# JOBR0/PerceiverIO_Pytorch

Measured on AMD Instinct MI355X. Metric: samples/sec PerceiverIO fwd (ImageNet-224, 512x1024 latents, 8 blocks x 6 self-attends), higher is better.
Workload: dtype f16; 1 GPU; imagenet224 ClassificationPerceiver (conv+Fourier prep -> encoder 3136x322->512x1024, 8x6 SA -> decoder 1000 queries -> final Linear), all rows computed; batch_per_gpu=32, global_batch=32, precision_policy=fp16x2w/fp16sd/fp16x2af, parallelism=dp1 (batch sharded, all-gather of logits), launch=one HIP graph replay per step

## Files before the change

include/pio_hip.h:

```cpp
#ifndef PIO_HIP_H
#define PIO_HIP_H

#include <stddef.h>
#include <stdint.h>

#ifdef __cplusplus
extern "C" {
#endif

#define PIO_VERSION 100

enum {
    PIO_OK = 0,
    PIO_E_SHAPE = -1,
    PIO_E_ALIGN = -2,
    PIO_E_ARCH = -3,
    PIO_E_WORKSPACE = -4,
    PIO_E_LAUNCH = -5,
    PIO_E_ARG = -6,
    PIO_E_RANGE = -7
};

enum { PIO_DT_F16 = 0, PIO_DT_BF16 = 1 };


typedef struct pio_linear_t {
    const void *w_hi;
    const void *w_lo;
    const float *bias;
    int32_t n;
    int32_t k;
    int32_t lo_row0;
} pio_linear_t;

typedef struct pio_layernorm_t {
    const float *gamma;
    const float *beta;
    int32_t c;
    float eps;
} pio_layernorm_t;

typedef struct pio_attention_t {
    pio_linear_t q, k, v, o;
    int32_t heads;
    int32_t dk, dv;
    int32_t dkp, dvp;
    int32_t q_in, k_in, v_in, out;
    int32_t dtype;
    int32_t act_split;
    pio_linear_t qk;
    pio_linear_t qkv;
    pio_linear_t kq, vo;
} pio_attention_t;

typedef struct pio_mlp_t {
    pio_linear_t fc1, fc2;
    int32_t in, hidden, out;
    int32_t dtype;
    int32_t act_split;
} pio_mlp_t;

typedef struct pio_ln_fold_t {
    pio_linear_t qkv;
    const float *qkv_c;
    pio_linear_t fc1;
    const float *fc1_c;
    int32_t *range_flag;
} pio_ln_fold_t;

typedef struct pio_self_attention_t {
    pio_layernorm_t ln1, ln2;
    pio_attention_t attn;
    pio_mlp_t mlp;
    pio_ln_fold_t fold;
} pio_self_attention_t;

typedef struct pio_cross_attention_t {
    pio_layernorm_t ln_q, ln_kv, ln2;
    pio_attention_t attn;
    pio_mlp_t mlp;
    int32_t use_query_residual;
} pio_cross_attention_t;

typedef struct pio_tensor3_t {
    const float *data;
    int64_t stride_b;
    int64_t stride_t;
    int32_t B, T, C;
} pio_tensor3_t;

int pio_version(void);
int pio_arch_ok(void);
const char *pio_error_string(int code);

#define PIO_PROF_CLASSES 9
int pio_prof_begin(int32_t max_records);
int pio_prof_end(double *ms, double *flops, double *bytes, int64_t *launches);

int pio_ln_fold_enable(int on);

int pio_gemm_kernel_override(int which);

int pio_stream_create_cu_mask(void **stream, const uint32_t *mask, uint32_t words);
int pio_stream_destroy(void *stream);
int pio_set_cu_budget(int32_t n_cu);

int32_t pio_pad8(int32_t c);
int32_t pio_padc(int32_t c);
size_t pio_packed_weight_bytes(int32_t out, int32_t in, int32_t row_heads, int32_t col_heads);
int pio_pack_linear(const float *w, const float *bias, int32_t out, int32_t in, int64_t ldw,
                    int32_t row_heads, int32_t col_heads, void *dst_hi, void *dst_lo, float *dst_bias,
                    int32_t dst_row0, int32_t k_pad, int32_t dtype, void *stream);

int pio_layernorm_cast(const pio_tensor3_t *x, const pio_layernorm_t *ln, void *y, void *y_lo, int32_t c_pad,
                       int32_t dtype, void *stream);

int pio_layernorm_cast_cat(const pio_tensor3_t *x1, const pio_tensor3_t *x2, const pio_layernorm_t *ln, void *y,
                           void *y_lo, int32_t c_pad, int32_t dtype, void *stream);

int pio_bn_relu_maxpool_tokens(const float *x, const float *scale, const float *shift, float *y, int32_t B, int32_t C,
                               int32_t H, int32_t W, int32_t pad_top, int32_t pad_left, void *stream);

typedef struct pio_gemm_t {
    const void *A, *B;
    const void *A_lo, *B_lo;
    void *C;
    void *C_lo;
    int32_t M, N, K;
    int64_t lda, ldb, ldc;
    int32_t batch, nh;
    int64_t sAb, sAh, sBb, sBh, sCb, sCh;
    const float *bias;
    int32_t bias_mode;
    int32_t act;
    float alpha;
    const float *R;
    int64_t ldr, r_stride_b;
    int32_t r_rows_per_batch;
    int32_t out_f32;
    int32_t n_store;
    int32_t dtype;
    void *X16;
    int64_t ld16;
    float *row_part;
    const float *ln_part;
    const float *ln_c;
    float ln_eps;
    void *X16_lo;
    const void *R16_hi, *R16_lo;
    int32_t b_lo_n0;
    int32_t *range_flag;
    int32_t ln_slots;
    int32_t row_slot_w;
} pio_gemm_t;
int pio_gemm_nt(const pio_gemm_t *g, void *stream);

int pio_softmax_rows(const float *S, int64_t lds, void *P, void *P_lo, int64_t ldp, int32_t B, int32_t H,
                     int32_t Tq, int32_t Tk, float scale, const uint8_t *kv_mask, const uint8_t *q_mask,
                     const uint8_t *full_mask, const float *bias, int32_t dtype, void *stream);

int pio_flash_attention(int32_t dtype, int32_t dkp, int32_t dvp, int32_t dk, const void *Q, const void *K, const void *V,
                        void *O, int32_t B, int32_t H, int32_t Tq, int32_t Tk, int64_t ldq, int64_t ldk, int64_t ldv,
                        int64_t ldo, int64_t sQb, int64_t sKb, int64_t sVb, int64_t sOb, int32_t v_rowmajor, void *stream);

size_t pio_flash_attention_pair_workspace_bytes(int32_t dkp, int32_t dvp, int32_t B, int32_t H, int32_t Tq, int32_t Tk);
int pio_flash_attention_pair(int32_t dtype, int32_t dkp, int32_t dvp, int32_t dk, const void *Q, const void *Q_lo,
                             const void *K, const void *K_lo, const void *V, void *O, void *O_lo, int32_t B, int32_t H,
                             int32_t Tq, int32_t Tk, int64_t ldq, int64_t ldk, int64_t ldv, int64_t ldo, int64_t sQb,
                             int64_t sKb, int64_t sVb, int64_t sOb, int32_t v_rowmajor, const uint8_t *kv_mask,
                             const uint8_t *q_mask, int32_t core, void *workspace, size_t workspace_bytes, void *stream);

size_t pio_attention_workspace_bytes(const pio_attention_t *a, int32_t B, int32_t Tq, int32_t Tk);
int pio_attention_fwd(const pio_attention_t *a, const pio_tensor3_t *inputs_q, const pio_tensor3_t *inputs_k,
                      const pio_tensor3_t *inputs_v, const uint8_t *kv_mask, const uint8_t *q_mask,
                      const uint8_t *full_mask, const float *attention_bias, float *out, float *probs_out,
                      void *workspace, size_t workspace_bytes, void *stream);

size_t pio_mlp_workspace_bytes(const pio_mlp_t *m, int64_t rows);
int pio_mlp_fwd(const pio_mlp_t *m, const pio_tensor3_t *x, float *out, void *workspace,
                size_t workspace_bytes, void *stream);

typedef struct pio_call_opts_t {
    int32_t ln_fold;
    int32_t cu_budget;
} pio_call_opts_t;

size_t pio_self_attention_workspace_bytes(const pio_self_attention_t *s, int32_t B, int32_t N);
int pio_self_attention_fwd(const pio_self_attention_t *s, const pio_tensor3_t *x, const uint8_t *kv_mask,
                           const uint8_t *q_mask, const uint8_t *full_mask, const float *attention_bias,
                           float *out, float *probs_out, void *workspace, size_t workspace_bytes, void *stream);

int pio_self_attention_fwd_opts(const pio_self_attention_t *s, const pio_tensor3_t *x, const uint8_t *kv_mask,
                                const uint8_t *q_mask, const uint8_t *full_mask, const float *attention_bias,
                                float *out, float *probs_out, void *workspace, size_t workspace_bytes, void *stream,
                                const pio_call_opts_t *opts);

size_t pio_cross_attention_workspace_bytes(const pio_cross_attention_t *c, int32_t B, int32_t Tq, int32_t Tk);
int pio_cross_attention_fwd(const pio_cross_attention_t *c, const pio_tensor3_t *inputs_q,
                            const pio_tensor3_t *inputs_kv, const uint8_t *kv_mask, const uint8_t *q_mask,
                            const uint8_t *full_mask, const float *attention_bias, float *out, float *probs_out,
                            void *workspace, size_t workspace_bytes, void *stream);

size_t pio_encoder_workspace_bytes(const pio_cross_attention_t *cross, const pio_self_attention_t *layers,
                                   int32_t L, int32_t B, int32_t M, int32_t N);
int pio_encoder_fwd(const pio_cross_attention_t *cross, const pio_self_attention_t *layers, int32_t L,
                    int32_t num_blocks, const pio_tensor3_t *inputs, const pio_tensor3_t *latents,
                    const uint8_t *input_mask, float *out, void *workspace, size_t workspace_bytes,
                    void *stream);

int pio_encoder_fwd_split(const pio_cross_attention_t *cross, const pio_self_attention_t *layers, int32_t L,
                          int32_t num_blocks, const pio_tensor3_t *inputs, const pio_tensor3_t *inputs_tail,
                          const pio_tensor3_t *latents, const uint8_t *input_mask, float *out, void *workspace,
                          size_t workspace_bytes, void *stream);

int pio_encoder_fwd_blocks(const pio_cross_attention_t *cross, const pio_self_attention_t *layers, int32_t L,
                           int32_t num_blocks, int32_t per_block, const pio_tensor3_t *inputs,
                           const pio_tensor3_t *inputs_tail, const pio_tensor3_t *latents, const uint8_t *input_mask,
                           float *out, void *workspace, size_t workspace_bytes, void *stream);

int pio_encoder_fwd_opts(const pio_cross_attention_t *cross, const pio_self_attention_t *layers, int32_t L,
                         int32_t num_blocks, int32_t per_block, const pio_tensor3_t *inputs,
                         const pio_tensor3_t *inputs_tail, const pio_tensor3_t *latents, const uint8_t *input_mask,
                         float *out, void *workspace, size_t workspace_bytes, void *stream,
                         const pio_call_opts_t *opts);

size_t pio_decoder_workspace_bytes(const pio_cross_attention_t *cross, const pio_linear_t *final_layer,
                                   int32_t B, int32_t Q, int32_t N);
int pio_decoder_fwd(const pio_cross_attention_t *cross, const pio_linear_t *final_layer, int32_t final_out,
                    const pio_tensor3_t *query, const pio_tensor3_t *latents, const uint8_t *query_mask,
                    float *out, void *workspace, size_t workspace_bytes, void *stream);

size_t pio_decoder_qcache_bytes(const pio_cross_attention_t *cross, int32_t Bq, int32_t Q);
int pio_decoder_fwd_qcache(const pio_cross_attention_t *cross, const pio_linear_t *final_layer, int32_t final_out,
                           const pio_tensor3_t *query, const pio_tensor3_t *latents, const uint8_t *query_mask,
                           float *out, void *workspace, size_t workspace_bytes, void *stream, void *q16_hi,
                           void *q16_lo, int32_t q16_valid);

int pio_decoder_fwd_split(const pio_cross_attention_t *cross, const pio_linear_t *final_layer, int32_t final_out,
                          const pio_tensor3_t *query, const pio_tensor3_t *query_tail, const pio_tensor3_t *latents,
                          const uint8_t *query_mask, float *out, void *workspace, size_t workspace_bytes, void *stream);

#ifdef __cplusplus
}
#endif
#endif
```

perceiverio_pytorch_amd/_lib.py:

```python
from __future__ import annotations

import ctypes as C
import os
import subprocess

_HERE = os.path.dirname(os.path.abspath(__file__))
LIB_PATH = os.environ.get("PIO_LIB_PATH", os.path.join(_HERE, "libpio_hip.so"))
CSRC = os.path.join(_HERE, "csrc")

PIO_DT_F16 = 0
PIO_DT_BF16 = 1

PIO_OK = 0
_ERRORS = {-1: "PIO_E_SHAPE", -2: "PIO_E_ALIGN", -3: "PIO_E_ARCH", -4: "PIO_E_WORKSPACE", -5: "PIO_E_LAUNCH",
           -6: "PIO_E_ARG", -7: "PIO_E_RANGE"}


class PioError(RuntimeError):
    pass


class Linear(C.Structure):
    _fields_ = [("w_hi", C.c_void_p), ("w_lo", C.c_void_p), ("bias", C.c_void_p), ("n", C.c_int32), ("k", C.c_int32),
                ("lo_row0", C.c_int32)]


class LayerNorm(C.Structure):
    _fields_ = [("gamma", C.c_void_p), ("beta", C.c_void_p), ("c", C.c_int32), ("eps", C.c_float)]


class Attention(C.Structure):
    _fields_ = [("q", Linear), ("k", Linear), ("v", Linear), ("o", Linear), ("heads", C.c_int32),
                ("dk", C.c_int32), ("dv", C.c_int32), ("dkp", C.c_int32), ("dvp", C.c_int32),
                ("q_in", C.c_int32), ("k_in", C.c_int32), ("v_in", C.c_int32), ("out", C.c_int32), ("dtype", C.c_int32),
                ("act_split", C.c_int32), ("qk", Linear), ("qkv", Linear), ("kq", Linear), ("vo", Linear)]


class Mlp(C.Structure):
    _fields_ = [("fc1", Linear), ("fc2", Linear), ("in_", C.c_int32), ("hidden", C.c_int32), ("out", C.c_int32),
                ("dtype", C.c_int32), ("act_split", C.c_int32)]


class LnFold(C.Structure):
    _fields_ = [("qkv", Linear), ("qkv_c", C.c_void_p), ("fc1", Linear), ("fc1_c", C.c_void_p),
                ("range_flag", C.c_void_p)]


class SelfAttention(C.Structure):
    _fields_ = [("ln1", LayerNorm), ("ln2", LayerNorm), ("attn", Attention), ("mlp", Mlp), ("fold", LnFold)]


class CrossAttention(C.Structure):
    _fields_ = [("ln_q", LayerNorm), ("ln_kv", LayerNorm), ("ln2", LayerNorm), ("attn", Attention), ("mlp", Mlp),
                ("use_query_residual", C.c_int32)]


class Tensor3(C.Structure):
    _fields_ = [("data", C.c_void_p), ("stride_b", C.c_int64), ("stride_t", C.c_int64), ("B", C.c_int32),
                ("T", C.c_int32), ("C", C.c_int32)]


class CallOpts(C.Structure):
    _fields_ = [("ln_fold", C.c_int32), ("cu_budget", C.c_int32)]


class Gemm(C.Structure):
    _fields_ = [("A", C.c_void_p), ("B", C.c_void_p), ("A_lo", C.c_void_p), ("B_lo", C.c_void_p), ("C", C.c_void_p),
                ("C_lo", C.c_void_p),
                ("M", C.c_int32), ("N", C.c_int32), ("K", C.c_int32),
                ("lda", C.c_int64), ("ldb", C.c_int64), ("ldc", C.c_int64),
                ("batch", C.c_int32), ("nh", C.c_int32),
                ("sAb", C.c_int64), ("sAh", C.c_int64), ("sBb", C.c_int64), ("sBh", C.c_int64),
                ("sCb", C.c_int64), ("sCh", C.c_int64),
                ("bias", C.c_void_p), ("bias_mode", C.c_int32), ("act", C.c_int32), ("alpha", C.c_float),
                ("R", C.c_void_p), ("ldr", C.c_int64), ("r_stride_b", C.c_int64),
                ("r_rows_per_batch", C.c_int32), ("out_f32", C.c_int32), ("n_store", C.c_int32),
                ("dtype", C.c_int32),
                ("X16", C.c_void_p), ("ld16", C.c_int64), ("row_part", C.c_void_p), ("ln_part", C.c_void_p),
                ("ln_c", C.c_void_p), ("ln_eps", C.c_float),
                ("X16_lo", C.c_void_p), ("R16_hi", C.c_void_p), ("R16_lo", C.c_void_p), ("b_lo_n0", C.c_int32),
                ("range_flag", C.c_void_p), ("ln_slots", C.c_int32), ("row_slot_w", C.c_int32)]


P = C.POINTER
_vp, _i32, _i64, _sz, _f = C.c_void_p, C.c_int32, C.c_int64, C.c_size_t, C.c_float
SIGNATURES = {
    "pio_version": (C.c_int, []),
    "pio_arch_ok": (C.c_int, []),
    "pio_error_string": (C.c_char_p, [C.c_int]),
    "pio_prof_begin": (C.c_int, [_i32]),
    "pio_prof_end": (C.c_int, [P(C.c_double), P(C.c_double), P(C.c_double), P(C.c_int64)]),
    "pio_pad8": (_i32, [_i32]),
    "pio_padc": (_i32, [_i32]),
    "pio_gemm_kernel_override": (C.c_int, [C.c_int]),
    "pio_ln_fold_enable": (C.c_int, [C.c_int]),
    "pio_stream_create_cu_mask": (C.c_int, [P(_vp), P(C.c_uint32), C.c_uint32]),
    "pio_stream_destroy": (C.c_int, [_vp]),
    "pio_set_cu_budget": (C.c_int, [_i32]),
    "pio_packed_weight_bytes": (_sz, [_i32, _i32, _i32, _i32]),
    "pio_pack_linear": (C.c_int, [_vp, _vp, _i32, _i32, _i64, _i32, _i32, _vp, _vp, _vp, _i32, _i32, _i32, _vp]),
    "pio_layernorm_cast": (C.c_int, [P(Tensor3), P(LayerNorm), _vp, _vp, _i32, _i32, _vp]),
    "pio_layernorm_cast_cat": (C.c_int, [P(Tensor3), P(Tensor3), P(LayerNorm), _vp, _vp, _i32, _i32, _vp]),
    "pio_bn_relu_maxpool_tokens": (C.c_int, [_vp, _vp, _vp, _vp, _i32, _i32, _i32, _i32, _i32, _i32, _vp]),
    "pio_gemm_nt": (C.c_int, [P(Gemm), _vp]),
    "pio_softmax_rows": (C.c_int, [_vp, _i64, _vp, _vp, _i64, _i32, _i32, _i32, _i32, _f, _vp, _vp, _vp, _vp, _i32, _vp]),
    "pio_flash_attention": (C.c_int, [_i32, _i32, _i32, _i32, _vp, _vp, _vp, _vp, _i32, _i32, _i32, _i32, _i64, _i64, _i64,
                                      _i64, _i64, _i64, _i64, _i64, _i32, _vp]),
    "pio_flash_attention_pair_workspace_bytes": (_sz, [_i32, _i32, _i32, _i32, _i32, _i32]),
    "pio_flash_attention_pair": (C.c_int, [_i32, _i32, _i32, _i32, _vp, _vp, _vp, _vp, _vp, _vp, _vp, _i32, _i32, _i32, _i32,
                                           _i64, _i64, _i64, _i64, _i64, _i64, _i64, _i64, _i32, _vp, _vp, _i32, _vp, _sz,
                                           _vp]),
    "pio_attention_workspace_bytes": (_sz, [P(Attention), _i32, _i32, _i32]),
    "pio_attention_fwd": (C.c_int, [P(Attention), P(Tensor3), P(Tensor3), P(Tensor3), _vp, _vp, _vp, _vp, _vp, _vp,
                                    _vp, _sz, _vp]),
    "pio_mlp_workspace_bytes": (_sz, [P(Mlp), _i64]),
    "pio_mlp_fwd": (C.c_int, [P(Mlp), P(Tensor3), _vp, _vp, _sz, _vp]),
    "pio_self_attention_workspace_bytes": (_sz, [P(SelfAttention), _i32, _i32]),
    "pio_self_attention_fwd": (C.c_int, [P(SelfAttention), P(Tensor3), _vp, _vp, _vp, _vp, _vp, _vp, _vp, _sz, _vp]),
    "pio_self_attention_fwd_opts": (C.c_int, [P(SelfAttention), P(Tensor3), _vp, _vp, _vp, _vp, _vp, _vp, _vp, _sz, _vp,
                                              P(CallOpts)]),
    "pio_cross_attention_workspace_bytes": (_sz, [P(CrossAttention), _i32, _i32, _i32]),
    "pio_cross_attention_fwd": (C.c_int, [P(CrossAttention), P(Tensor3), P(Tensor3), _vp, _vp, _vp, _vp, _vp, _vp,
                                          _vp, _sz, _vp]),
    "pio_encoder_workspace_bytes": (_sz, [P(CrossAttention), P(SelfAttention), _i32, _i32, _i32, _i32]),
    "pio_encoder_fwd": (C.c_int, [P(CrossAttention), P(SelfAttention), _i32, _i32, P(Tensor3), P(Tensor3), _vp, _vp,
                                  _vp, _sz, _vp]),
    "pio_encoder_fwd_split": (C.c_int, [P(CrossAttention), P(SelfAttention), _i32, _i32, P(Tensor3), P(Tensor3),
                                        P(Tensor3), _vp, _vp, _vp, _sz, _vp]),
    "pio_encoder_fwd_blocks": (C.c_int, [P(CrossAttention), P(SelfAttention), _i32, _i32, _i32, P(Tensor3), P(Tensor3),
                                         P(Tensor3), _vp, _vp, _vp, _sz, _vp]),
    "pio_encoder_fwd_opts": (C.c_int, [P(CrossAttention), P(SelfAttention), _i32, _i32, _i32, P(Tensor3), P(Tensor3),
                                       P(Tensor3), _vp, _vp, _vp, _sz, _vp, P(CallOpts)]),
    "pio_decoder_workspace_bytes": (_sz, [P(CrossAttention), P(Linear), _i32, _i32, _i32]),
    "pio_decoder_fwd": (C.c_int, [P(CrossAttention), P(Linear), _i32, P(Tensor3), P(Tensor3), _vp, _vp, _vp, _sz,
                                  _vp]),
    "pio_decoder_qcache_bytes": (_sz, [P(CrossAttention), _i32, _i32]),
    "pio_decoder_fwd_qcache": (C.c_int, [P(CrossAttention), P(Linear), _i32, P(Tensor3), P(Tensor3), _vp, _vp, _vp, _sz,
                                         _vp, _vp, _vp, _i32]),
    "pio_decoder_fwd_split": (C.c_int, [P(CrossAttention), P(Linear), _i32, P(Tensor3), P(Tensor3), P(Tensor3), _vp, _vp, _vp,
                                        _sz, _vp]),
}

_lib = None


def build(verbose: bool = False) -> str:
    out = subprocess.run(["make", "-C", CSRC, "-j8"], capture_output=True, text=True)
    if verbose or out.returncode:
        print(out.stdout[-4000:])
        print(out.stderr[-4000:])
    if out.returncode:
        raise PioError("building libpio_hip.so failed")
    return LIB_PATH


def lib() -> C.CDLL:
    global _lib
    if _lib is None:
        if not os.path.exists(LIB_PATH):
            raise PioError(f"{LIB_PATH} is missing: run `python -c 'import __graft_entry__ as g; g.build()'` "
                           "(there is no CPU / eager fallback for the PerceiverIO hot path)")
        l = C.CDLL(LIB_PATH)
        for name, (res, args) in SIGNATURES.items():
            fn = getattr(l, name)
            fn.restype = res
            fn.argtypes = args
        _lib = l
    return _lib


def check(code: int, what: str = "") -> None:
    if code != PIO_OK:
        raise PioError(f"{what}: {_ERRORS.get(code, code)}")
```

perceiverio_pytorch_amd/csrc/pio_flash.hip:

```cpp
#include <stdio.h>
#include <stdlib.h>

#include <type_traits>

#include "pio_internal.h"

namespace pio {

#ifndef PIO_FLASH_DEFAULT_VARIANT
#define PIO_FLASH_DEFAULT_VARIANT 0
#endif

struct FlashParams {
    const void *Q, *K, *VT;
    void *O;
    int Tq, Tk, H, nqt;
    int64_t ldq, ldk, ldvt, ldo;
    int64_t sQb, sKb, sVb, sOb;
    float scale_log2;
    int o_rows16;
    const void *Q_lo, *K_lo;
    void *O_lo;
};

static __device__ __attribute__((aligned(16))) uint32_t g_zero_chunk_f[4] = {0, 0, 0, 0};

template <int DV>
__device__ __forceinline__ int vrow_swz(int r) {
    if constexpr (DV == 128) return ((r & 3) << 2) | ((r >> 2) & 3);
    else if constexpr (DV == 64) return ((r >> 1) & 1) << 2;
    else return 0;
}

template <int DT, int DK, int DV, bool VROW, int NW, int KS = 1, bool QK_PAIR = false>
__global__ __launch_bounds__(NW * 64, NW >= 8 ? 1 : 2) void flash_attn_kernel(const FlashParams p) {
    static_assert(!QK_PAIR || (DK == 32 && DT == PIO_DT_F16), "pair-operand Q K^T: the DK = 32 fp16 instantiations");
    typedef typename Op<DT>::T T;
    typedef typename Op<DT>::V8 V8;
    typedef typename Op<DT>::V4 V4;
    typedef short tr4 __attribute__((__vector_size__(4 * sizeof(short))));
    static_assert(!VROW || DV == 128 || DV == 64 || DV == 32 || DV == 160, "row-major V: swizzles exist for these widths");
    constexpr int KT = 64;
    constexpr int K_TILE = KT * DK * 2;
    constexpr int K_STG = QK_PAIR ? 2 * K_TILE : K_TILE;
    constexpr int V_TILE = DV * KT * 2;
    constexpr int KCPR = DK / 8;
    constexpr int KRPB = 16 / KCPR;
    constexpr int K_PIECES = K_TILE / 1024;
    constexpr int V_PIECES = V_TILE / 1024;
    constexpr int NDT = DV / 32;
    constexpr int NQS = DK / 16;
    constexpr int OROW = DV * 2 + 16;
    static_assert(KS == 1 || ((KS == 2 || KS == 4) && NW == 4 * KS), "key split: KS groups of four waves");
    constexpr int NWQ = NW / KS;
    constexpr int MRG = KS > 1 ? (KS - 1) * NWQ * 64 * (NDT * 16 + 2) * 4 : 0;
    constexpr int RING = 2 * KS * (K_STG + V_TILE), OSTG = NW * 32 * OROW;
    constexpr int SM0 = RING > OSTG ? RING : OSTG;
    __shared__ __attribute__((aligned(16))) char smem[SM0 > MRG ? SM0 : MRG];

    const int tid = threadIdx.x;
    const int lane = tid & 63;
    const int wave = __builtin_amdgcn_readfirstlane(tid >> 6);
    const int r32 = lane & 31, hh = lane >> 5;
    int bid = blockIdx.x;
    const int nblk = gridDim.x;
    if ((nblk & 7) == 0) bid = (bid & 7) * (nblk >> 3) + (bid >> 3);
    const int qt = bid % p.nqt, bh = bid / p.nqt;
    const int b = bh / p.H, h = bh % p.H;
    const int qb = KS == 1 ? wave : wave % NWQ, kh = KS == 1 ? 0 : wave / NWQ;
    const int q0 = qt * (NWQ * 32) + qb * 32;

    const T *Qg = (const T *)p.Q + b * p.sQb + (int64_t)h * DK;
    const T *Kg = (const T *)p.K + b * p.sKb + (int64_t)h * DK;
    const T *Vg = (const T *)p.VT + b * p.sVb + (VROW ? (int64_t)h * DV : (int64_t)h * DV * p.ldvt);
    const T *zsrc = (const T *)g_zero_chunk_f;
    const T *Klg = nullptr;
    if constexpr (QK_PAIR) Klg = (const T *)p.K_lo + b * p.sKb + (int64_t)h * DK;

    V8 qf[NQS];
    V8 ql[QK_PAIR ? NQS : 1];

    const int ntiles_all = (p.Tk + KT - 1) / KT;
    const int ntiles = ntiles_all / KS;
    const int tile0 = kh * ntiles;

    auto stage = [&](int kt, int buf) {
        char *kb = smem + (buf * KS + kh) * (K_STG + V_TILE);
        char *vb = kb + K_STG;
        const int k0 = (tile0 + kt) * KT;
        for (int pc = qb; pc < K_PIECES; pc += NWQ) {
            const int row = pc * (64 / KCPR) + lane / KCPR;
            const int slot = lane % KCPR;
            const int c = slot ^ ((row / KRPB) & (KCPR - 1));
            int key = k0 + row;
            key = key < p.Tk ? key : p.Tk - 1;
            const T *src = Kg + (int64_t)key * p.ldk + c * 8;
            __builtin_amdgcn_global_load_lds((const __attribute__((address_space(1))) void *)src,
                                             (__attribute__((address_space(3))) void *)(kb + pc * 1024), 16, 0, 0);
            if constexpr (QK_PAIR)
                __builtin_amdgcn_global_load_lds(
                    (const __attribute__((address_space(1))) void *)(Klg + (int64_t)key * p.ldk + c * 8),
                    (__attribute__((address_space(3))) void *)(kb + K_TILE + pc * 1024), 16, 0, 0);
        }
        if constexpr (VROW) {
            constexpr int VCPR = DV / 8;
            for (int pc = qb; pc < V_PIECES; pc += NWQ) {
                const int idx = pc * 64 + lane;
                const int row = idx / VCPR;
                const int slot = idx - row * VCPR;
                const int c = slot ^ vrow_swz<DV>(row);
                int key = k0 + row;
                key = key < p.Tk ? key : p.Tk - 1;
                const T *src = Vg + (int64_t)key * p.ldvt + c * 8;
                __builtin_amdgcn_global_load_lds((const __attribute__((address_space(1))) void *)src,
                                                 (__attribute__((address_space(3))) void *)(vb + pc * 1024), 16, 0,
                                                 0);
            }
        } else
        for (int pc = qb; pc < V_PIECES; pc += NWQ) {
            const int row = pc * 8 + (lane >> 3);
            const int slot = lane & 7;
            const int c = slot ^ ((row >> 1) & 7);
            const int kcol = k0 + c * 8;
            const T *src = (kcol < p.ldvt) ? Vg + (int64_t)row * p.ldvt + kcol : zsrc;
            __builtin_amdgcn_global_load_lds((const __attribute__((address_space(1))) void *)src,
                                             (__attribute__((address_space(3))) void *)(vb + pc * 1024), 16, 0, 0);
        }
    };

    f32x16 oacc[NDT];
#pragma unroll
    for (int i = 0; i < NDT; ++i)
#pragma unroll
        for (int j = 0; j < 16; ++j) oacc[i][j] = 0.f;
    float m_run = -INFINITY;
    float l_run = 0.f;

    int k_off[2];
#pragma unroll
    for (int t = 0; t < 2; ++t) k_off[t] = (32 * t + r32) * (DK * 2);
    const int k_swz = (r32 / KRPB) & (KCPR - 1);
    const int v_swz = (r32 >> 1) & 7;

    stage(0, 0);
    {
        int q = q0 + r32;
        q = q < p.Tq ? q : p.Tq - 1;
        const T *qrow = Qg + (int64_t)q * p.ldq + 8 * hh;
#pragma unroll
        for (int s = 0; s < NQS; ++s) qf[s] = *(const V8 *)(qrow + 16 * s);
        if constexpr (QK_PAIR) {
            const T *lrow = (const T *)p.Q_lo + b * p.sQb + (int64_t)h * DK + (int64_t)q * p.ldq + 8 * hh;
#pragma unroll
            for (int s = 0; s < NQS; ++s) ql[s] = *(const V8 *)(lrow + 16 * s);
        }
    }
    for (int kt = 0; kt < ntiles; ++kt) {
        asm volatile("s_waitcnt vmcnt(0)" ::: "memory");
        __syncthreads();
        if (kt + 1 < ntiles) stage(kt + 1, (kt + 1) & 1);
        const char *kb = smem + ((kt & 1) * KS + kh) * (K_STG + V_TILE);
        const char *vb = kb + K_STG;

        f32x16 sacc[2];
#pragma unroll
        for (int t = 0; t < 2; ++t) {
#pragma unroll
            for (int j = 0; j < 16; ++j) sacc[t][j] = 0.f;
            if constexpr (QK_PAIR) {
                V8 kh_f[NQS], kl_f[NQS];
#pragma unroll
                for (int s = 0; s < NQS; ++s) {
                    const int chunk = (2 * s + hh) ^ k_swz;
                    kh_f[s] = *(const V8 *)(kb + k_off[t] + chunk * 16);
                    kl_f[s] = *(const V8 *)(kb + K_TILE + k_off[t] + chunk * 16);
                }
#pragma unroll
                for (int s = 0; s < NQS; ++s) sacc[t] = Op<DT>::mfma32(kl_f[s], qf[s], sacc[t]);
#pragma unroll
                for (int s = 0; s < NQS; ++s) sacc[t] = Op<DT>::mfma32(kh_f[s], ql[s], sacc[t]);
#pragma unroll
                for (int s = 0; s < NQS; ++s) sacc[t] = Op<DT>::mfma32(kh_f[s], qf[s], sacc[t]);
            } else
#pragma unroll
            for (int s = 0; s < NQS; ++s) {
                const int chunk = (2 * s + hh) ^ k_swz;
                const V8 kf = *(const V8 *)(kb + k_off[t] + chunk * 16);
                sacc[t] = Op<DT>::mfma32(kf, qf[s], sacc[t]);
            }
        }
        const bool tail = KS == 1 && (kt == ntiles - 1) && (p.Tk % KT != 0);
        float mx = -INFINITY;
        if (tail) {
#pragma unroll
            for (int t = 0; t < 2; ++t)
#pragma unroll
                for (int i = 0; i < 16; ++i) {
                    const int key = (tile0 + kt) * KT + 32 * t + (i & 3) + 8 * (i >> 2) + 4 * hh;
                    if (key >= p.Tk) sacc[t][i] = -INFINITY;
                }
        }
#pragma unroll
        for (int t = 0; t < 2; ++t)
#pragma unroll
            for (int i = 0; i < 16; ++i) mx = fmaxf(mx, sacc[t][i]);
        mx = fmaxf(mx, __shfl_xor(mx, 32, 64)) * p.scale_log2;
        const float m_new = fmaxf(m_run, mx);
        const float alpha = __builtin_amdgcn_exp2f(m_run - m_new);
        m_run = m_new;
        float psum = 0.f;
#pragma unroll
        for (int t = 0; t < 2; ++t)
#pragma unroll
            for (int i = 0; i < 16; ++i) {
                const float e = __builtin_amdgcn_exp2f(fmaf(sacc[t][i], p.scale_log2, -m_new));
                sacc[t][i] = e;
                psum += e;
            }
        l_run = l_run * alpha + psum;
        if (__builtin_amdgcn_ballot_w64(alpha != 1.0f) != 0) {
#pragma unroll
            for (int d = 0; d < NDT; ++d)
#pragma unroll
                for (int j = 0; j < 16; ++j) oacc[d][j] *= alpha;
        }

        V8 pf[2][2];
#pragma unroll
        for (int t = 0; t < 2; ++t)
#pragma unroll
            for (int s = 0; s < 2; ++s)
#pragma unroll
                for (int j = 0; j < 8; ++j) pf[t][s][j] = Op<DT>::from_f32(sacc[t][8 * s + j]);

#pragma unroll
        for (int d = 0; d < NDT; ++d) {
            const char *vrow = vb + (32 * d + r32) * 128;
#pragma unroll
            for (int t = 0; t < 2; ++t)
#pragma unroll
                for (int s = 0; s < 2; ++s) {
                    V4 lo, hi;
                    if constexpr (VROW) {
                        const int q4 = (lane & 15) >> 2, p4 = lane & 3, g1 = (lane >> 4) & 1;
                        const int chunk = d * 4 + 2 * g1 + (p4 >> 1);
#pragma unroll
                        for (int jj = 0; jj < 2; ++jj) {
                            const int key = 32 * t + 16 * s + 8 * jj + 4 * hh + q4;
                            const int f = vrow_swz<DV>(key);
                            const char *a = vb + key * (DV * 2) + ((chunk ^ f) << 4) + 8 * (p4 & 1);
                            const tr4 r = __builtin_amdgcn_ds_read_tr16_b64_v4i16(
                                (__attribute__((address_space(3))) tr4 *)a);
                            if (jj == 0) lo = __builtin_bit_cast(V4, r);
                            else hi = __builtin_bit_cast(V4, r);
                        }
                    } else {
                        const int g = 8 * t + 4 * s + hh;
                        lo = *(const V4 *)(vrow + ((((g >> 1)) ^ v_swz) << 4) + (g & 1) * 8);
                        hi = *(const V4 *)(vrow + ((((g + 2) >> 1) ^ v_swz) << 4) + (g & 1) * 8);
                    }
                    V8 vf;
#pragma unroll
                    for (int j = 0; j < 4; ++j) {
                        vf[j] = lo[j];
                        vf[4 + j] = hi[j];
                    }
                    oacc[d] = Op<DT>::mfma32(vf, pf[t][s], oacc[d]);
                }
        }
    }

    if constexpr (KS > 1) {
        __syncthreads();
        constexpr int MW = NDT * 16 + 2;
        if (kh > 0) {
            float *mg = (float *)smem + (size_t)(((kh - 1) * NWQ + qb) * 64 + lane) * MW;
#pragma unroll
            for (int d = 0; d < NDT; ++d)
#pragma unroll
                for (int j = 0; j < 16; ++j) mg[d * 16 + j] = oacc[d][j];
            mg[NDT * 16] = m_run;
            mg[NDT * 16 + 1] = l_run;
        }
        __syncthreads();
        if (kh == 0) {
#pragma unroll
            for (int part = 1; part < KS; ++part) {
                const float *mg = (const float *)smem + (size_t)(((part - 1) * NWQ + qb) * 64 + lane) * MW;
                const float m1 = mg[NDT * 16], l1 = mg[NDT * 16 + 1];
                const float m = fmaxf(m_run, m1);
                const float a0 = __builtin_amdgcn_exp2f(m_run - m), a1 = __builtin_amdgcn_exp2f(m1 - m);
#pragma unroll
                for (int d = 0; d < NDT; ++d)
#pragma unroll
                    for (int j = 0; j < 16; ++j) oacc[d][j] = oacc[d][j] * a0 + mg[d * 16 + j] * a1;
                l_run = l_run * a0 + l1 * a1;
                m_run = m;
            }
        }
    }
    const float l_tot = l_run + __shfl_xor(l_run, 32, 64);
    const float inv = 1.0f / l_tot;
    if (p.o_rows16) {
        __syncthreads();
        if (kh != 0) return;
        char *const ost = smem + qb * (32 * OROW);
        char *const orow = ost + r32 * OROW;
#pragma unroll
        for (int d = 0; d < NDT; ++d)
#pragma unroll
            for (int g4 = 0; g4 < 4; ++g4) {
                V4 o;
#pragma unroll
                for (int j = 0; j < 4; ++j) o[j] = Op<DT>::from_f32(oacc[d][4 * g4 + j] * inv);
                *(V4 *)(orow + (32 * d + 8 * g4 + 4 * hh) * 2) = o;
            }
        constexpr int CPR = DV / 8;
        T *const og = (T *)p.O + b * p.sOb + (int64_t)h * DV;
#pragma unroll
        for (int idx0 = 0; idx0 < 32 * CPR; idx0 += 64) {
            const int idx = idx0 + lane;
            const int row = idx / CPR, ch = idx % CPR;
            if (idx < 32 * CPR && q0 + row < p.Tq)
                *(V8 *)(og + (int64_t)(q0 + row) * p.ldo + ch * 8) = *(const V8 *)(ost + row * OROW + ch * 16);
        }
        return;
    }
    const int q = q0 + r32;
    if (q < p.Tq && kh == 0) {
        T *orow = (T *)p.O + b * p.sOb + (int64_t)q * p.ldo + (int64_t)h * DV;
#pragma unroll
        for (int d = 0; d < NDT; ++d)
#pragma unroll
            for (int g4 = 0; g4 < 4; ++g4) {
                V4 o;
#pragma unroll
                for (int j = 0; j < 4; ++j) o[j] = Op<DT>::from_f32(oacc[d][4 * g4 + j] * inv);
                *(V4 *)(orow + 32 * d + 8 * g4 + 4 * hh) = o;
                if constexpr (QK_PAIR) {
                    if (p.O_lo) {
                        V4 l;
#pragma unroll
                        for (int j = 0; j < 4; ++j)
                            l[j] = Op<DT>::from_f32(oacc[d][4 * g4 + j] * inv - Op<DT>::to_f32(o[j]));
                        *(V4 *)((T *)p.O_lo + (orow - (T *)p.O) + 32 * d + 8 * g4 + 4 * hh) = l;
                    }
                }
            }
    }
}

#ifdef PIO_EXPERIMENTS
#include "../../tools/experiments/pio_flash_variants.inc"
#endif

#ifdef PIO_EXPERIMENTS
int flash_variant_override(int which) {
    static int cur = [] {
        const char *e = getenv("PIO_FLASH_VARIANT");
        const int v = e ? atoi(e) : PIO_FLASH_DEFAULT_VARIANT;
        return (v >= 0 && v <= 2) ? v : PIO_FLASH_DEFAULT_VARIANT;
    }();
    const int prev = cur;
    if (which >= 0 && which <= 2) cur = which;
    return prev;
}
extern "C" int pio_debug_flash_variant(int which) { return flash_variant_override(which); }
#endif

template <int DT, int DK, int DV, bool PAIR>
static void flash_launch(const FlashRoute &r, dim3 grid, hipStream_t s, const FlashParams &p) {
    void (*k)(FlashParams) = flash_attn_kernel<DT, DK, DV, false, 4, 1, PAIR>;
    if (r.v_rowmajor) k = flash_attn_kernel<DT, DK, DV, true, 4, 1, PAIR>;
    if (r.NW == 8) k = r.KS == 2 ? flash_attn_kernel<DT, DK, DV, true, 8, 2, PAIR> : flash_attn_kernel<DT, DK, DV, true, 8, 1, PAIR>;
    if constexpr (DK <= 64 && DV <= 64)
        if (r.NW == 16) k = flash_attn_kernel<DT, DK, DV, true, 16, 4, PAIR>;
    hipLaunchKernelGGL(k, grid, dim3(r.threads), 0, s, p);
}
template <int DK, int DV>
static void flash_launch_dt(int dtype, bool pair, const FlashRoute &r, dim3 grid, hipStream_t s, const FlashParams &p) {
    if constexpr (DK == 32)
        if (pair) return flash_launch<PIO_DT_F16, DK, DV, true>(r, grid, s, p);
    if (dtype == PIO_DT_F16) flash_launch<PIO_DT_F16, DK, DV, false>(r, grid, s, p);
    else flash_launch<PIO_DT_BF16, DK, DV, false>(r, grid, s, p);
}

int flash_attention_launch(int dtype, int dkp, int dvp, int dk_logical, const AttnOperands &t, int B, int H, int Tq, int Tk,
                           bool v_rowmajor, hipStream_t s) {
    if (!flash_supported(dkp, dvp)) return PIO_E_SHAPE;
    if (attn_operands_present(t) != PIO_OK) return PIO_E_ARG;
    const bool pair = t.Q_lo != nullptr;
    if (t.O_lo && !pair) return PIO_E_ARG;
    if (pair && !flash_pair_supported(dtype, dkp, dvp)) return PIO_E_SHAPE;
    if (B <= 0 || H <= 0 || Tq <= 0 || Tk <= 0 || (int64_t)B * H * ((Tq + 127) / 128) > 0x7fffffffLL) return PIO_E_SHAPE;
    if (attn_operands_aligned(t) != PIO_OK) return PIO_E_ALIGN;
    static const bool ksplit_on = [] {
        const char *e = getenv("PIO_FLASH_KSPLIT");
        return !e || atoi(e) != 0;
    }();
    const FlashRoute r = flash_route(dkp, dvp, B, H, Tq, Tk, v_rowmajor, ksplit_on, cu_budget());
    const int o_rows16 = (!t.O_lo && t.ldo % 8 == 0 && t.sOb % 8 == 0 && ((uintptr_t)t.O & 15) == 0) ? 1 : 0;
    FlashParams p{t.Q, t.K, t.VT, t.O, Tq, Tk, H, r.nqt, t.ldq, t.ldk, t.ldvt, t.ldo, t.sQb, t.sKb, t.sVb, t.sOb,
                  1.4426950408889634f / sqrtf((float)dk_logical), o_rows16, t.Q_lo, t.K_lo, t.O_lo};
    dim3 grid((unsigned)(r.nqt * B * H), 1, 1);
    ProfScope prof(PROF_FLASH, 2.0 * B * H * (double)Tq * Tk * (dkp + dvp),
                   2.0 * B * H * ((double)Tq * (dkp + dvp) + (double)Tk * (dkp + dvp)), s);
    int variant = 0;
#ifdef PIO_EXPERIMENTS
    variant = flash_variant_override(-2);
#endif
    static const bool debug = [] {
        const char *e = getenv("PIO_FLASH_DEBUG");
        return e && atoi(e) != 0;
    }();
    if (debug)
        fprintf(stderr, "[pio] fused attention B=%d H=%d Tq=%d Tk=%d dkp=%d dvp=%d v_rowmajor=%d NW=%d KS=%d variant=%d\n", B,
                H, Tq, Tk, dkp, dvp, (int)v_rowmajor, r.NW, r.KS, variant);
#ifdef PIO_EXPERIMENTS
    if (!pair && v_rowmajor && Tq >= 256 && Tk % 128 == 0 && variant == 1 && o_rows16) {
        FlashParams pp = p;
        pp.nqt = (Tq + 255) / 256;
        dim3 pgrid((unsigned)(pp.nqt * B * H), 1, 1);
        if (dtype == PIO_DT_F16) hipLaunchKernelGGL((flash_attn_pipe_kernel<PIO_DT_F16>), pgrid, dim3(256), 0, s, pp);
        else hipLaunchKernelGGL((flash_attn_pipe_kernel<PIO_DT_BF16>), pgrid, dim3(256), 0, s, pp);
        return launch_status();
    }
    if (!pair && r.NW == 8 && r.KS == 1 && variant == 2) {
        if (dtype == PIO_DT_F16) hipLaunchKernelGGL((flash_attn_stag_kernel<PIO_DT_F16>), grid, dim3(512), 0, s, p);
        else hipLaunchKernelGGL((flash_attn_stag_kernel<PIO_DT_BF16>), grid, dim3(512), 0, s, p);
        return launch_status();
    }
#endif
    if (dkp == 128) flash_launch_dt<128, 128>(dtype, pair, r, grid, s, p);
    else if (dkp == 64) flash_launch_dt<64, 64>(dtype, pair, r, grid, s, p);
    else if (dvp == 32) flash_launch_dt<32, 32>(dtype, pair, r, grid, s, p);
    else flash_launch_dt<32, 160>(dtype, pair, r, grid, s, p);
    return launch_status();
}

}
```

Measured before the change: 2012 samples/s.

## Split flash softmax into 32-key halves and interleave exp with PV MFMAs

Adds a HALVES variant of the flash attention kernel. It runs the online softmax over each 32-key half of the 64-key tile separately and overlaps the second half's exponentials with the first half's P·V MFMAs, using sched_barriers to pin the order. The intent is to hide the exp/VALU latency of the softmax behind matrix-core work. This path is on by default for non-pair, KS=1 routes, and variant 3 restores the old path. The cost is an extra rescale of the accumulators per tile and higher register pressure.

Result: no change. 2005 samples/s (-0.4%).

```diff
diff --git a/include/pio_hip.h b/include/pio_hip.h
--- a/include/pio_hip.h
+++ b/include/pio_hip.h
@@ -100,6 +100,9 @@
 int pio_ln_fold_enable(int on);
 
 int pio_gemm_kernel_override(int which);
+
+int pio_debug_flash_variant(int which);
+int pio_debug_flash_last_kernel(void);
 
 int pio_stream_create_cu_mask(void **stream, const uint32_t *mask, uint32_t words);
 int pio_stream_destroy(void *stream);
diff --git a/perceiverio_pytorch_amd/_lib.py b/perceiverio_pytorch_amd/_lib.py
--- a/perceiverio_pytorch_amd/_lib.py
+++ b/perceiverio_pytorch_amd/_lib.py
@@ -93,6 +93,8 @@
     "pio_pad8": (_i32, [_i32]),
     "pio_padc": (_i32, [_i32]),
     "pio_gemm_kernel_override": (C.c_int, [C.c_int]),
+    "pio_debug_flash_variant": (C.c_int, [C.c_int]),
+    "pio_debug_flash_last_kernel": (C.c_int, []),
     "pio_ln_fold_enable": (C.c_int, [C.c_int]),
     "pio_stream_create_cu_mask": (C.c_int, [P(_vp), P(C.c_uint32), C.c_uint32]),
     "pio_stream_destroy": (C.c_int, [_vp]),
diff --git a/perceiverio_pytorch_amd/csrc/pio_flash.hip b/perceiverio_pytorch_amd/csrc/pio_flash.hip
--- a/perceiverio_pytorch_amd/csrc/pio_flash.hip
+++ b/perceiverio_pytorch_amd/csrc/pio_flash.hip
@@ -32,9 +32,16 @@
     else return 0;
 }
 
-template <int DT, int DK, int DV, bool VROW, int NW, int KS = 1, bool QK_PAIR = false>
+__device__ __forceinline__ float vmax_f32(float a, float b) {
+    float r;
+    asm("v_max_f32 %0, %1, %2" : "=v"(r) : "v"(a), "v"(b));
+    return r;
+}
+
+template <int DT, int DK, int DV, bool VROW, int NW, int KS = 1, bool QK_PAIR = false, bool HALVES = false>
 __global__ __launch_bounds__(NW * 64, NW >= 8 ? 1 : 2) void flash_attn_kernel(const FlashParams p) {
     static_assert(!QK_PAIR || (DK == 32 && DT == PIO_DT_F16), "pair-operand Q K^T: the DK = 32 fp16 instantiations");
+    static_assert(!HALVES || (KS == 1 && !QK_PAIR), "32-key softmax steps: the single-part, single-operand kernels");
     typedef typename Op<DT>::T T;
     typedef typename Op<DT>::V8 V8;
     typedef typename Op<DT>::V4 V4;
@@ -142,6 +149,7 @@
     const int k_swz = (r32 / KRPB) & (KCPR - 1);
     const int v_swz = (r32 >> 1) & 7;
 
+    const int xlane32 = (lane ^ 32) << 2;
     stage(0, 0);
     {
         int q = q0 + r32;
@@ -189,8 +197,37 @@
                 sacc[t] = Op<DT>::mfma32(kf, qf[s], sacc[t]);
             }
         }
+        auto v_frag = [&](int d, int t, int s) {
+            V4 lo, hi;
+            if constexpr (VROW) {
+                const int q4 = (lane & 15) >> 2, p4 = lane & 3, g1 = (lane >> 4) & 1;
+                const int chunk = d * 4 + 2 * g1 + (p4 >> 1);
+#pragma unroll
+                for (int jj = 0; jj < 2; ++jj) {
+                    const int key = 32 * t + 16 * s + 8 * jj + 4 * hh + q4;
+                    const int f = vrow_swz<DV>(key);
+                    const char *a = vb + key * (DV * 2) + ((chunk ^ f) << 4) + 8 * (p4 & 1);
+                    const tr4 r = __builtin_amdgcn_ds_read_tr16_b64_v4i16(
+                        (__attribute__((address_space(3))) tr4 *)a);
+                    if (jj == 0) lo = __builtin_bit_cast(V4, r);
+                    else hi = __builtin_bit_cast(V4, r);
+                }
+            } else {
+                const char *vrow = vb + (32 * d + r32) * 128;
+                const int g = 8 * t + 4 * s + hh;
+                lo = *(const V4 *)(vrow + ((((g >> 1)) ^ v_swz) << 4) + (g & 1) * 8);
+                hi = *(const V4 *)(vrow + ((((g + 2) >> 1) ^ v_swz) << 4) + (g & 1) * 8);
+            }
+            V8 vf;
+#pragma unroll
+            for (int j = 0; j < 4; ++j) {
+                vf[j] = lo[j];
+                vf[4 + j] = hi[j];
+            }
+            return vf;
+        };
+        auto pv_step = [&](int d, int t, int s, const V8 &pfrag) { oacc[d] = Op<DT>::mfma32(v_frag(d, t, s), pfrag, oacc[d]); };
         const bool tail = KS == 1 && (kt == ntiles - 1) && (p.Tk % KT != 0);
-        float mx = -INFINITY;
         if (tail) {
 #pragma unroll
             for (int t = 0; t < 2; ++t)
@@ -200,73 +237,116 @@
                     if (key >= p.Tk) sacc[t][i] = -INFINITY;
                 }
         }
-#pragma unroll
-        for (int t = 0; t < 2; ++t)
-#pragma unroll
-            for (int i = 0; i < 16; ++i) mx = fmaxf(mx, sacc[t][i]);
-        mx = fmaxf(mx, __shfl_xor(mx, 32, 64)) * p.scale_log2;
-        const float m_new = fmaxf(m_run, mx);
-        const float alpha = __builtin_amdgcn_exp2f(m_run - m_new);
-        m_run = m_new;
-        float psum = 0.f;
-#pragma unroll
-        for (int t = 0; t < 2; ++t)
-#pragma unroll
-            for (int i = 0; i < 16; ++i) {
+        if constexpr (HALVES) {
+            auto half_max = [&](int t) {
+                float mx = -INFINITY;
+#pragma unroll
+                for (int i = 0; i < 16; ++i) mx = fmaxf(mx, sacc[t][i]);
+                const float mo = __builtin_bit_cast(float, __builtin_amdgcn_ds_bpermute(xlane32, __builtin_bit_cast(int, mx)));
+                return vmax_f32(mx, mo) * p.scale_log2;
+            };
+            auto exp_elem = [&](int t, int i, float m_new, float &psum) {
                 const float e = __builtin_amdgcn_exp2f(fmaf(sacc[t][i], p.scale_log2, -m_new));
                 sacc[t][i] = e;
                 psum += e;
-            }
-        l_run = l_run * alpha + psum;
-        if (__builtin_amdgcn_ballot_w64(alpha != 1.0f) != 0) {
+            };
+            auto p_frag = [&](int t, int s) {
+                V8 f;
+#pragma unroll
+                for (int j = 0; j < 8; ++j) f[j] = Op<DT>::from_f32(sacc[t][8 * s + j]);
+                return f;
+            };
+            auto rescale = [&](float alpha) {
+                if (__builtin_amdgcn_ballot_w64(alpha != 1.0f) != 0) {
+#pragma unroll
+                    for (int d = 0; d < NDT; ++d)
+#pragma unroll
+                        for (int j = 0; j < 16; ++j) oacc[d][j] *= alpha;
+                }
+            };
+            const float m0 = vmax_f32(m_run, half_max(0));
+            const float a0 = __builtin_amdgcn_exp2f(m_run - m0);
+            rescale(a0);
+            const float m1 = vmax_f32(m0, half_max(1));
+            const float a1 = __builtin_amdgcn_exp2f(m0 - m1);
+            m_run = m1;
+            float ps0 = 0.f, ps1 = 0.f;
+            V8 pf0[2], pf1[2];
+#pragma unroll
+            for (int i = 0; i < 8; ++i) exp_elem(0, i, m0, ps0);
+            pf0[0] = p_frag(0, 0);
+            constexpr int NG = 2 * NDT, E0 = (8 + NDT - 1) / NDT, E1 = (16 + NG - 1) / NG;
+            V8 vf = v_frag(0, 0, 0);
+            __builtin_amdgcn_sched_barrier(0);
+#pragma unroll
+            for (int g = 0; g < NG; ++g) {
+                const int d = g % NDT, s = g / NDT;
+                V8 vn = vf;
+                if (g + 1 < NG) vn = v_frag((g + 1) % NDT, 0, (g + 1) / NDT);
+                if (g == NDT) pf0[1] = p_frag(0, 1);
+                oacc[d] = Op<DT>::mfma32(vf, pf0[s], oacc[d]);
+#pragma unroll
+                for (int j = 0; j < E0; ++j)
+                    if (g < NDT && 8 + g * E0 + j < 16) exp_elem(0, 8 + g * E0 + j, m0, ps0);
+#pragma unroll
+                for (int j = 0; j < E1; ++j)
+                    if (g * E1 + j < 16) exp_elem(1, g * E1 + j, m1, ps1);
+#pragma unroll
+                for (int j = 0; j < E1; ++j)
+                    if (g * E1 + j < 16) asm volatile("" ::"v"(sacc[1][g * E1 + j]));
+                asm volatile("" ::"v"(ps0), "v"(ps1));
+                vf = vn;
+                __builtin_amdgcn_sched_barrier(0);
+            }
+            l_run = (l_run * a0 + ps0) * a1 + ps1;
+            pf1[0] = p_frag(1, 0);
+            pf1[1] = p_frag(1, 1);
+            rescale(a1);
 #pragma unroll
             for (int d = 0; d < NDT; ++d)
 #pragma unroll
-                for (int j = 0; j < 16; ++j) oacc[d][j] *= alpha;
-        }
-
-        V8 pf[2][2];
-#pragma unroll
-        for (int t = 0; t < 2; ++t)
-#pragma unroll
-            for (int s = 0; s < 2; ++s)
-#pragma unroll
-                for (int j = 0; j < 8; ++j) pf[t][s][j] = Op<DT>::from_f32(sacc[t][8 * s + j]);
-
-#pragma unroll
-        for (int d = 0; d < NDT; ++d) {
-            const char *vrow = vb + (32 * d + r32) * 128;
+                for (int s = 0; s < 2; ++s) pv_step(d, 1, s, pf1[s]);
+        } else {
+            float mx = -INFINITY;
 #pragma unroll
             for (int t = 0; t < 2; ++t)
 #pragma unroll
-                for (int s = 0; s < 2; ++s) {
-                    V4 lo, hi;
-                    if constexpr (VROW) {
-                        const int q4 = (lane & 15) >> 2, p4 = lane & 3, g1 = (lane >> 4) & 1;
-                        const int chunk = d * 4 + 2 * g1 + (p4 >> 1);
-#pragma unroll
-                        for (int jj = 0; jj < 2; ++jj) {
-                            const int key = 32 * t + 16 * s + 8 * jj + 4 * hh + q4;
-                            const int f = vrow_swz<DV>(key);
-                            const char *a = vb + key * (DV * 2) + ((chunk ^ f) << 4) + 8 * (p4 & 1);
-                            const tr4 r = __builtin_amdgcn_ds_read_tr16_b64_v4i16(
-                                (__attribute__((address_space(3))) tr4 *)a);
-                            if (jj == 0) lo = __builtin_bit_cast(V4, r);
-                            else hi = __builtin_bit_cast(V4, r);
-                        }
-                    } else {
-                        const int g = 8 * t + 4 * s + hh;
-                        lo = *(const V4 *)(vrow + ((((g >> 1)) ^ v_swz) << 4) + (g & 1) * 8);
-                        hi = *(const V4 *)(vrow + ((((g + 2) >> 1) ^ v_swz) << 4) + (g & 1) * 8);
-                    }
-                    V8 vf;
-#pragma unroll
-                    for (int j = 0; j < 4; ++j) {
-                        vf[j] = lo[j];
-                        vf[4 + j] = hi[j];
-                    }
-                    oacc[d] = Op<DT>::mfma32(vf, pf[t][s], oacc[d]);
+                for (int i = 0; i < 16; ++i) mx = fmaxf(mx, sacc[t][i]);
+            mx = fmaxf(mx, __shfl_xor(mx, 32, 64)) * p.scale_log2;
+            const float m_new = fmaxf(m_run, mx);
+            const float alpha = __builtin_amdgcn_exp2f(m_run - m_new);
+            m_run = m_new;
+            float psum = 0.f;
+#pragma unroll
+            for (int t = 0; t < 2; ++t)
+#pragma unroll
+                for (int i = 0; i < 16; ++i) {
+                    const float e = __builtin_amdgcn_exp2f(fmaf(sacc[t][i], p.scale_log2, -m_new));
+                    sacc[t][i] = e;
+                    psum += e;
                 }
+            l_run = l_run * alpha + psum;
+            if (__builtin_amdgcn_ballot_w64(alpha != 1.0f) != 0) {
+#pragma unroll
+                for (int d = 0; d < NDT; ++d)
+#pragma unroll
+                    for (int j = 0; j < 16; ++j) oacc[d][j] *= alpha;
+            }
+
+            V8 pf[2][2];
+#pragma unroll
+            for (int t = 0; t < 2; ++t)
+#pragma unroll
+                for (int s = 0; s < 2; ++s)
+#pragma unroll
+                    for (int j = 0; j < 8; ++j) pf[t][s][j] = Op<DT>::from_f32(sacc[t][8 * s + j]);
+
+#pragma unroll
+            for (int d = 0; d < NDT; ++d)
+#pragma unroll
+                for (int t = 0; t < 2; ++t)
+#pragma unroll
+                    for (int s = 0; s < 2; ++s) pv_step(d, t, s, pf[t][s]);
         }
     }
 
@@ -354,35 +434,49 @@
 #include "../../tools/experiments/pio_flash_variants.inc"
 #endif
 
+static bool flash_variant_known(int v) {
 #ifdef PIO_EXPERIMENTS
+    return v >= 0 && v <= 3;
+#else
+    return v == 0 || v == 3;
+#endif
+}
+static int g_flash_last_kernel = 0;
 int flash_variant_override(int which) {
     static int cur = [] {
         const char *e = getenv("PIO_FLASH_VARIANT");
         const int v = e ? atoi(e) : PIO_FLASH_DEFAULT_VARIANT;
-        return (v >= 0 && v <= 2) ? v : PIO_FLASH_DEFAULT_VARIANT;
+        return flash_variant_known(v) ? v : PIO_FLASH_DEFAULT_VARIANT;
     }();
     const int prev = cur;
-    if (which >= 0 && which <= 2) cur = which;
+    if (flash_variant_known(which)) cur = which;
     return prev;
 }
 extern "C" int pio_debug_flash_variant(int which) { return flash_variant_override(which); }
-#endif
+extern "C" int pio_debug_flash_last_kernel(void) { return g_flash_last_kernel; }
 
 template <int DT, int DK, int DV, bool PAIR>
-static void flash_launch(const FlashRoute &r, dim3 grid, hipStream_t s, const FlashParams &p) {
-    void (*k)(FlashParams) = flash_attn_kernel<DT, DK, DV, false, 4, 1, PAIR>;
-    if (r.v_rowmajor) k = flash_attn_kernel<DT, DK, DV, true, 4, 1, PAIR>;
-    if (r.NW == 8) k = r.KS == 2 ? flash_attn_kernel<DT, DK, DV, true, 8, 2, PAIR> : flash_attn_kernel<DT, DK, DV, true, 8, 1, PAIR>;
+static void flash_launch(const FlashRoute &r, bool halves, dim3 grid, hipStream_t s, const FlashParams &p) {
+    constexpr bool HV = !PAIR;
+    halves = halves && HV && r.KS == 1;
+    void (*k)(FlashParams) = halves ? flash_attn_kernel<DT, DK, DV, false, 4, 1, PAIR, HV> : flash_attn_kernel<DT, DK, DV, false, 4, 1, PAIR>;
+    if (r.v_rowmajor) k = halves ? flash_attn_kernel<DT, DK, DV, true, 4, 1, PAIR, HV> : flash_attn_kernel<DT, DK, DV, true, 4, 1, PAIR>;
+    if (r.NW == 8) {
+        if (r.KS == 2) k = flash_attn_kernel<DT, DK, DV, true, 8, 2, PAIR>;
+        else k = halves ? flash_attn_kernel<DT, DK, DV, true, 8, 1, PAIR, HV> : flash_attn_kernel<DT, DK, DV, true, 8, 1, PAIR>;
+    }
     if constexpr (DK <= 64 && DV <= 64)
         if (r.NW == 16) k = flash_attn_kernel<DT, DK, DV, true, 16, 4, PAIR>;
+    g_flash_last_kernel = (r.NW << 8) | (r.KS << 4) | ((PAIR ? 1 : 0) << 1) | (halves ? 1 : 0);
     hipLaunchKernelGGL(k, grid, dim3(r.threads), 0, s, p);
 }
 template <int DK, int DV>
-static void flash_launch_dt(int dtype, bool pair, const FlashRoute &r, dim3 grid, hipStream_t s, const FlashParams &p) {
+static void flash_launch_dt(int dtype, bool pair, const FlashRoute &r, bool halves, dim3 grid, hipStream_t s,
+                            const FlashParams &p) {
     if constexpr (DK == 32)
-        if (pair) return flash_launch<PIO_DT_F16, DK, DV, true>(r, grid, s, p);
-    if (dtype == PIO_DT_F16) flash_launch<PIO_DT_F16, DK, DV, false>(r, grid, s, p);
-    else flash_launch<PIO_DT_BF16, DK, DV, false>(r, grid, s, p);
+        if (pair) return flash_launch<PIO_DT_F16, DK, DV, true>(r, halves, grid, s, p);
+    if (dtype == PIO_DT_F16) flash_launch<PIO_DT_F16, DK, DV, false>(r, halves, grid, s, p);
+    else flash_launch<PIO_DT_BF16, DK, DV, false>(r, halves, grid, s, p);
 }
 
 int flash_attention_launch(int dtype, int dkp, int dvp, int dk_logical, const AttnOperands &t, int B, int H, int Tq, int Tk,
@@ -405,10 +499,7 @@
     dim3 grid((unsigned)(r.nqt * B * H), 1, 1);
     ProfScope prof(PROF_FLASH, 2.0 * B * H * (double)Tq * Tk * (dkp + dvp),
                    2.0 * B * H * ((double)Tq * (dkp + dvp) + (double)Tk * (dkp + dvp)), s);
-    int variant = 0;
-#ifdef PIO_EXPERIMENTS
-    variant = flash_variant_override(-2);
-#endif
+    const int variant = flash_variant_override(-2);
     static const bool debug = [] {
         const char *e = getenv("PIO_FLASH_DEBUG");
         return e && atoi(e) != 0;
@@ -431,10 +522,11 @@
         return launch_status();
     }
 #endif
-    if (dkp == 128) flash_launch_dt<128, 128>(dtype, pair, r, grid, s, p);
-    else if (dkp == 64) flash_launch_dt<64, 64>(dtype, pair, r, grid, s, p);
-    else if (dvp == 32) flash_launch_dt<32, 32>(dtype, pair, r, grid, s, p);
-    else flash_launch_dt<32, 160>(dtype, pair, r, grid, s, p);
+    const bool halves = variant != 3;
+    if (dkp == 128) flash_launch_dt<128, 128>(dtype, pair, r, halves, grid, s, p);
+    else if (dkp == 64) flash_launch_dt<64, 64>(dtype, pair, r, halves, grid, s, p);
+    else if (dvp == 32) flash_launch_dt<32, 32>(dtype, pair, r, halves, grid, s, p);
+    else flash_launch_dt<32, 160>(dtype, pair, r, halves, grid, s, p);
     return launch_status();
 }
 
```
